# Chuanming-Liu/DAzimSurfTomo

Hardware: AMD Instinct MI355X
Metric: FMM traveltime fields/sec (256^2 grid, 16 periods) + LSQR SpMV HBM GB/s (higher is better)
Workload: dtype f32

## Files before the change

dazimsurftomo_amd/csrc/rays.hip:

```cpp
#include <cmath>
#include <chrono>
#include <unistd.h>

#include "dazim_internal.h"

#include <rocprim/device/device_scan.hpp>
#include <rocprim/device/device_radix_sort.hpp>

namespace {

constexpr int GDX = 5, GDZ = 5;
constexpr int RM = DAZIM_RMAX;
constexpr float EARTH = 6371.0f;
constexpr float FTOL = 1e-4f;

struct RayArgs {
  dazim_geom g;
  int nx, ny, nz, kmax;
  long nray;
  const int *field;
  const float *rcx, *rcz;
  const float *scx, *scz;
  const int *period;
  const int *kidx;
  const float *veln;
  const float *ttn;
  const int *tslot;
  int tsh;
  long fstride;
  const int *fdone;
  int *defer_mark;
  int max_quads;
  int sweeps;
  const float *ttnr;
  const int *nstsr;
  const dazim_refbox *boxes;
  const float *vels;
  const double *svs, *svp, *srho;
  unsigned nvx_magic;
  const double *skern;
  const float *lsen;
  double r_dnx, r_dnz, r_dnxr, r_dnzr, r_dvx, r_dvz, r_e2dnx, r_e2dnxr;
  float dplh;
  float *dsurf;
  int *status;
  int *rbflag;
  long *count;
  int *nlist;
  unsigned short *lcell;
  float *lval;
  float *fdm_scratch;
  int LK;
  int lcap;
  const unsigned *perm;
  unsigned *qcount;
  float2 *pts;
  int *npts;
  int pcap;
  int dense;
  long *countd;
  int keep_small;
  const long *rowptr;
  float *val;
  int *col;
};

__device__ __forceinline__ float dz_sinf(float x) {
  if (!(x > 0.0f && x < 3.1415927f)) return (float)sin((double)x);
  const double y = (double)x - 1.5707963267948966192;
  const double y2 = y * y;
  double p = -1.5619206968586226e-16;
  p = fma(p, y2, 4.7794773323873853e-14);
  p = fma(p, y2, -1.1470745597729725e-11);
  p = fma(p, y2, 2.0876756987868099e-09);
  p = fma(p, y2, -2.7557319223985891e-07);
  p = fma(p, y2, 2.4801587301587302e-05);
  p = fma(p, y2, -1.3888888888888889e-03);
  p = fma(p, y2, 4.1666666666666664e-02);
  p = fma(p, y2, -0.5);
  p = fma(p, y2, 1.0);
  return (float)p;
}

__device__ __forceinline__ void step_azimuth(float x0, float z0, float x1, float z1, float &c2psi, float &s2psi) {
  const float PI_F = 3.1415926535898f;
  const float evtlat = (PI_F / 2 - x0) * 180.0f / PI_F, evtlon = z0 * 180.0f / PI_F;
  const float stalat = (PI_F / 2 - x1) * 180.0f / PI_F, stalon = z1 * 180.0f / PI_F;
  const double pi = (double)3.1415926535898f;
  const float piby2 = (float)(pi / (double)2.f);
  const double rad = (double)2.f * pi / (double)360.f;
  const double sph = (double)(1.0f / 298.257f);
  const double scolat = (double)piby2 - atan((1. - sph) * (1. - sph) * tan((double)stalat * rad));
  const double ecolat = (double)piby2 - atan((1. - sph) * (1. - sph) * tan((double)evtlat * rad));
  const double slon = (double)stalon * rad, elon = (double)evtlon * rad;
  const double a = sin(scolat) * cos(slon), b = sin(scolat) * sin(slon), c = cos(scolat);
  const double dd = sin(elon), ee = -cos(elon), cc = cos(ecolat);
  const double gg = -cc * ee, hh = cc * dd, kk = -sin(ecolat);
  const double rhs1 = (a - dd) * (a - dd) + (b - ee) * (b - ee) + c * c - (double)2.f;
  const double rhs2 = (a - gg) * (a - gg) + (b - hh) * (b - hh) + (c - kk) * (c - kk) - (double)2.f;
  double daz = atan2(rhs1, rhs2);
  if (daz < 0.0) daz = daz + 2 * pi;
  float az = (float)(daz / rad);
  if (fabsf(az - 360.f) < .00001f) az = 0.0f;
  const float rgpsi = az / 180 * PI_F;
  c2psi = (float)cos((double)(2.0f * rgpsi));
  s2psi = (float)sin((double)(2.0f * rgpsi));
}

__device__ __forceinline__ float divr(float x, double rd) { return (float)((double)x * rd); }

__device__ __forceinline__ void basis(float v, float b[4]) {
  const float om = 1.0f - v;
  b[0] = om * om * om / 6.0f;
  b[1] = (4.0f - 6.0f * (v * v) + 3.0f * (v * v * v)) / 6.0f;
  b[2] = (1.0f + 3.0f * v + 3.0f * (v * v) - 3.0f * (v * v * v)) / 6.0f;
  b[3] = v * v * v / 6.0f;
}

__device__ __forceinline__ float div6(float x) { return divr(x, 1.0 / 6.0); }
__device__ __forceinline__ float basis1(float v, int i) {
  const float om = 1.0f - v;
  const float n0 = om * om * om;
  const float n1 = 4.0f - 6.0f * (v * v) + 3.0f * (v * v * v);
  const float n2 = 1.0f + 3.0f * v + 3.0f * (v * v) - 3.0f * (v * v * v);
  const float n3 = v * v * v;
  return div6(i == 0 ? n0 : (i == 1 ? n1 : (i == 2 ? n2 : n3)));
}

__device__ __forceinline__ float vel_at(const dazim_geom &g, const float *veln, int ipx, int ipz, float drx, float drz,
                                        double rdnx, double rdnz) {
  float vel = 0.0f;
#pragma unroll
  for (int l = 1; l <= 2; l++)
#pragma unroll
    for (int m = 1; m <= 2; m++) {
      float produ = (1.0f - fabsf(divr((float)(m - 1) * g.dnz - drz, rdnz)));
      produ = produ * (1.0f - fabsf(divr((float)(l - 1) * g.dnx - drx, rdnx)));
      if (ipz - 1 + m <= g.nnz && ipx - 1 + l <= g.nnx && ipz - 1 + m >= 1 && ipx - 1 + l >= 1)
        vel = vel + veln[(size_t)(ipx - 2 + l) * g.nnz + (ipz - 2 + m)] * produ;
    }
  return vel;
}

__device__ __forceinline__ float bilin_cell(const dazim_geom &g, const float *veln, int cx, int cz, float px, float pz,
                                            double rdnx, double rdnz) {
  const float drx = (px - g.gox) - (float)(cx - 1) * g.dnx;
  const float drz = (pz - g.goz) - (float)(cz - 1) * g.dnz;
  float biv = 0.0f;
#pragma unroll
  for (int i = 1; i <= 2; i++)
#pragma unroll
    for (int j = 1; j <= 2; j++) {
      const float produ = (1.0f - fabsf(divr((float)(i - 1) * g.dnx - drx, rdnx))) *
                          (1.0f - fabsf(divr((float)(j - 1) * g.dnz - drz, rdnz)));
      biv = biv + veln[(size_t)(cx - 2 + i) * g.nnz + (cz - 2 + j)] * produ;
    }
  return biv;
}

__global__ void k_row_kernels(long n, int kmax, long ncol, const float *__restrict__ vels, const double *__restrict__ svs,
                              const double *__restrict__ svp, const double *__restrict__ srho, double *__restrict__ out) {
  const long i = (long)blockIdx.x * blockDim.x + threadIdx.x;
  if (i >= n) return;
  const long k = i / (kmax * ncol), c = i % ncol;
  out[i] = dz_row_kernel(vels[k * ncol + c], svs[i], svp[i], srho[i]);
}

__global__ void k_ray_keys(long nray, const int *__restrict__ field, const float *__restrict__ scx, const float *__restrict__ scz,
                           const float *__restrict__ rcx, const float *__restrict__ rcz, float inv_dmax, int dbits,
                           unsigned *__restrict__ keys, unsigned *__restrict__ iota, const int *__restrict__ order) {
  const long i = (long)blockIdx.x * blockDim.x + threadIdx.x;
  if (i >= nray) return;
  const int f = field[i];
  const float dx = scx[f] - rcx[i], dz = (scz[f] - rcz[i]) * __sinf(rcx[i]);
  const float d = sqrtf(dx * dx + dz * dz) * inv_dmax;
  const unsigned dmaxq = (1u << dbits) - 1u;
  unsigned q = d >= 1.0f ? dmaxq : (unsigned)(d * (float)dmaxq);
  keys[i] = ((unsigned)(order ? order[f] : f) << dbits) | (dmaxq - q);
  iota[i] = (unsigned)i;
}

constexpr int GP_COUNT = 8, GP_EMIT = 16;
constexpr int RAYS_MINW = 4;
constexpr int RPW_MAX = 64 / GP_COUNT;
__device__ __forceinline__ void cbar() { asm volatile("" ::: "memory"); }

template <bool EMIT, bool AZIM, bool TILED, bool MAP>
__global__ __launch_bounds__(64, AZIM ? 2 : RAYS_MINW) void rays_kernel(RayArgs A_) {
  using ArgP = const __attribute__((address_space(4))) RayArgs *;
  auto launder = [](ArgP p) {
    int z;
    asm volatile("v_mov_b32 %0, 0" : "=v"(z));
    return (ArgP)((const __attribute__((address_space(4))) char *)p + __builtin_amdgcn_readfirstlane(z));
  };
  ArgP Ap = launder((ArgP)__builtin_amdgcn_kernarg_segment_ptr());
#define A (*Ap)
#define RAYS_ARGS_FRESH Ap = launder(Ap)
  constexpr int GP = EMIT ? GP_EMIT : GP_COUNT;
  constexpr int RPW = 64 / GP;
  constexpr int LPR = 16 / GP;
  constexpr int LSTEP = 4 / LPR;
  constexpr unsigned GMASK = (1u << GP) - 1u;
  extern __shared__ __attribute__((aligned(16))) unsigned short s_lists[];
  dazim_geom g;
  g.nvx = A.g.nvx; g.nvz = A.g.nvz; g.nnx = A.g.nnx; g.nnz = A.g.nnz;
  g.gox = A.g.gox; g.goz = A.g.goz; g.dnx = A.g.dnx; g.dnz = A.g.dnz; g.dvx = A.g.dvx; g.dvz = A.g.dvz;
  const int lane = threadIdx.x, grp = lane / GP, gl = lane & (GP - 1);
  const int lm = gl & 3, l0 = gl >> 2;
  const int nnx = g.nnx, nnz = g.nnz, nvx = g.nvx, nvz = g.nvz, ldf = nvz + 2, nf = ldf * (nvx + 2);
  constexpr int NG = AZIM ? 3 : 1;
  const unsigned nvx_magic = A.nvx_magic;
  const int LC = A.lcap;
  unsigned short *s_list = s_lists + (size_t)grp * LC;
  float *gfdm = A.fdm_scratch + ((size_t)blockIdx.x * RPW + grp) * nf * NG;
  float *gfdmc = gfdm + nf, *gfdms = gfdm + 2 * nf;
  const float gox = g.gox, goz = g.goz, dnx = g.dnx, dnz = g.dnz, dvx = g.dvx, dvz = g.dvz;
  const double rdnx = A.r_dnx, rdnz = A.r_dnz, rdnxr = A.r_dnxr, rdnzr = A.r_dnzr, rdvx = A.r_dvx, rdvz = A.r_dvz;
  const unsigned gmask_shift = grp * GP;
  const long nquad = (A.nray + RPW - 1) / RPW;
  const int nxcd = (gridDim.x % 8 == 0) ? 8 : 1;
  unsigned *qcnt = A.qcount + (EMIT ? 8 : 0);
  int chunk = (int)(blockIdx.x % nxcd);
  int traced = 0;
  for (;;) {
    RAYS_ARGS_FRESH;
    long quad = -1;
    if (lane == 0) {
      for (int tried = 0; tried < nxcd; tried++) {
        const long lo = nquad * chunk / nxcd, hi = nquad * (chunk + 1) / nxcd;
        const long b = lo < hi ? (long)atomicAdd(&qcnt[chunk], 1u) : hi;
        if (lo + b < hi) {
          quad = lo + b;
          break;
        }
        if (!EMIT && A.sweeps > 1 && lo < hi && b < (hi - lo) * A.sweeps) {
          quad = lo + b % (hi - lo);
          break;
        }
        chunk = (chunk + 1) % nxcd;
      }
    }
    quad = ((long)__shfl((int)(quad >> 32), 0) << 32) | (unsigned)__shfl((int)quad, 0);
    chunk = __shfl(chunk, 0);
    if (quad < 0) break;
    const long slot = quad * RPW + grp;
    if (!EMIT && A.defer_mark) {
      if (!A.defer_mark[quad]) continue;
      if (A.fdone) {
        const int fq = slot < A.nray ? A.field[A.perm ? (long)A.perm[slot] : slot] : -1;
        const int st = fq >= 0 ? __hip_atomic_load(A.fdone + fq, __ATOMIC_ACQUIRE, __HIP_MEMORY_SCOPE_AGENT) : 1;
        if (__ballot(st != 1) != 0) continue;
        __builtin_amdgcn_fence(__ATOMIC_ACQUIRE, "agent");
      }
      if (A.max_quads > 0 && traced >= A.max_quads) break;
      int mine = 0;
      if (lane == 0) mine = __hip_atomic_exchange(A.defer_mark + quad, 0, __ATOMIC_RELAXED, __HIP_MEMORY_SCOPE_AGENT);
      mine = __shfl(mine, 0);
      if (!mine) continue;
      traced++;
      if (lane == 0) atomicAdd(&A.qcount[18], 1u);
    }
    if (slot >= A.nray) continue;
    const long ray = A.perm ? (long)A.perm[slot] : slot;
    const int f = A.field[ray];
    const float scx = A.scx[f], scz = A.scz[f], rcx = A.rcx[ray], rcz = A.rcz[ray];
    const float *veln = A.veln + (size_t)(A.period[f] - 1) * nnx * nnz;
    const float *ttn = TILED ? A.ttn + (size_t)(A.tslot ? A.tslot[f] : f) * A.fstride : A.ttn + (size_t)f * nnx * nnz;
    const int tsh = TILED ? A.tsh : 0;
    auto tnode = [&](int x0, int z0) -> float {
      return TILED ? ttn[dz_tile_x(x0, tsh) + dz_tile_z(z0)] : ttn[(size_t)x0 * nnz + z0];
    };
    const float *ttnr = A.ttnr + (size_t)f * RM * RM;
    const int *nstsr = A.nstsr + (size_t)f * RM * RM;
    const dazim_refbox bx = A.boxes[f];
    const int saved = EMIT ? A.nlist[ray] : -1;
    if (saved < 0)
      for (int i = gl; i < nf * NG; i += GP) gfdm[i] = 0.0f;
    cbar();
    int status = 0, rb = 0;
    if (!EMIT) {
      int irx = (int)divr(rcx - gox, rdnx) + 1, irz = (int)divr(rcz - goz, rdnz) + 1;
      if (irx < 1 || irx > nnx || irz < 1 || irz > nnz) status = DAZIM_E_RECEIVER_OUTSIDE;
      if (!status) {
        if (irx == nnx) irx--;
        if (irz == nnz) irz--;
        const int isx = (int)divr(scx - gox, rdnx) + 1, isz = (int)divr(scz - goz, rdnz) + 1;
        float sred = ((scx - rcx) * EARTH) * ((scx - rcx) * EARTH);
        const float e2 = (scz - rcz) * EARTH * dz_sinf(rcx);
        sred = sqrtf(sred + e2 * e2);
        bool sw = sred < A.dplh;
        if (isx == irx && isz == irz) sw = true;
        float trr;
        if (sw) {
          const float vs = bilin_cell(g, veln, isx, isz, scx, scz, rdnx, rdnz);
          const float vr = bilin_cell(g, veln, irx, irz, rcx, rcz, rdnx, rdnz);
          trr = 2.0f * sred / (vs + vr);
        } else {
          const float drx = (rcx - gox) - (float)(irx - 1) * dnx;
          const float drz = (rcz - goz) - (float)(irz - 1) * dnz;
          trr = 0.0f;
#pragma unroll
          for (int k = 1; k <= 2; k++)
#pragma unroll
            for (int l = 1; l <= 2; l++) {
              const float produ = (1.0f - fabsf(divr((float)(l - 1) * dnz - drz, rdnz))) *
                                  (1.0f - fabsf(divr((float)(k - 1) * dnx - drx, rdnx)));
              trr = trr + tnode(irx - 2 + k, irz - 2 + l) * produ;
            }
        }
        if (gl == 0) A.dsurf[ray] = trr;
      }
    }
    const float goxr = bx.goxr, gozr = bx.gozr, dnxr = bx.dnxr, dnzr = bx.dnzr;
    const int nnxr = bx.nnxr, nnzr = bx.nnzr;
    const int isx = (int)divr(scx - goxr, rdnxr) + 1, isz = (int)divr(scz - gozr, rdnzr) + 1;
    const float dpl = 0.5f * A.dplh;
    int ipx = (int)divr(rcx - gox, rdnx) + 1, ipz = (int)divr(rcz - goz, rdnz) + 1;
    if (ipx < 1 || ipx >= nnx || ipz < 1 || ipz >= nnz) status = DAZIM_E_RECEIVER_OUTSIDE;
    if (!status && saved < 0) {
      float x0 = rcx, z0 = rcz;
      float sinx0 = dz_sinf(x0);
      int sw = 0;
      float sred = ((scx - x0) * EARTH) * ((scx - x0) * EARTH);
      float e2 = (scz - z0) * EARTH * sinx0;
      sred = sqrtf(sred + e2 * e2);
      if (sred < 2.0f * dpl) sw = 1;
      int ipxr = (int)divr(rcx - goxr, rdnxr) + 1, ipzr = (int)divr(rcz - gozr, rdnzr) + 1;
      auto in_refined = [&](int px, int pz) -> int {
        if (px < 1 || px >= nnxr || pz < 1 || pz >= nnzr) return 0;
        const int *sp = nstsr + (size_t)(px - 1) * RM + (pz - 1);
        if (sp[0] != 0 || sp[1] != 0) return 0;
        if (sp[RM] != 0 || sp[RM + 1] != 0) return 0;
        return 1;
      };
      int igref = in_refined(ipxr, ipzr);
      if (sw == 0 && igref == 1 && ipxr == isx && ipzr == isz) sw = 1;
      const bool keep_pts = !EMIT && A.pts != nullptr && gl == 0;
      float2 *rp = A.pts ? A.pts + (size_t)ray * A.pcap : nullptr;
      int np = 1;
      if (keep_pts) {
        rp[0] = make_float2(rcx, rcz);
        if (sw == 1) { if (A.pcap > 1) rp[1] = make_float2(scx, scz); np = 2; }
      }
      int cbx = -100, cbz = -100;
      float acc[LPR], accc[LPR], accs[LPR];
#pragma unroll
      for (int q = 0; q < LPR; q++) acc[q] = accc[q] = accs[q] = 0.0f;
      auto flush = [&]() {
        if (cbx > -100) {
#pragma unroll
          for (int q = 0; q < LPR; q++) {
            const int fi = (cbx + lm) * ldf + (cbz + l0 + q * LSTEP);
            gfdm[fi] = acc[q];
            if (AZIM) { gfdmc[fi] = accc[q]; gfdms[fi] = accs[q]; }
          }
        }
      };
      float tc00, tc01, tc10, tc11, tr00 = 0.0f, tr01 = 0.0f, tr10 = 0.0f, tr11 = 0.0f;
      auto load_corner_times = [&]() {
        if (TILED) {
          const int x0 = dz_tile_x(ipx - 1, tsh), x1 = dz_tile_x(ipx, tsh), z0 = dz_tile_z(ipz - 1), z1 = dz_tile_z(ipz);
          tc00 = ttn[x0 + z0]; tc01 = ttn[x0 + z1]; tc10 = ttn[x1 + z0]; tc11 = ttn[x1 + z1];
        } else {
          const float *t = ttn + (size_t)(ipx - 1) * nnz + (ipz - 1);
          tc00 = t[0]; tc01 = t[1]; tc10 = t[nnz]; tc11 = t[nnz + 1];
        }
        if (ipxr >= 1 && ipxr < nnxr && ipzr >= 1 && ipzr < nnzr) {
          const float *u = ttnr + (size_t)(ipxr - 1) * RM + (ipzr - 1);
          tr00 = u[0]; tr01 = u[1]; tr10 = u[RM]; tr11 = u[RM + 1];
        }
      };
      load_corner_times();
      bool carry = false;
      float vel_c = 0.0f, vi_c = 0.0f, wi_c[LPR];
#pragma unroll
      for (int q = 0; q < LPR; q++) wi_c[q] = 0.0f;
      const long maxrp = (long)nnx * nnz;
      for (long j = 1; j <= maxrp; j++) {
        if (sw == 1) break;
        float dtx, dtz;
        if (igref == 1) {
          dtx = tr10 - tr00;
          dtx = dtx + tr11 - tr01;
          dtx = divr(dtx, A.r_e2dnxr);
          dtz = tr01 - tr00;
          dtz = dtz + tr11 - tr10;
          dtz = dtz / (2.0f * EARTH * sinx0 * dnzr);
        } else {
          dtx = tc10 - tc00;
          dtx = dtx + tc11 - tc01;
          dtx = divr(dtx, A.r_e2dnx);
          dtz = tc01 - tc00;
          dtz = dtz + tc11 - tc10;
          dtz = dtz / (2.0f * EARTH * sinx0 * dnz);
        }
        const float rd1 = sqrtf(dtx * dtx + dtz * dtz);
        float x1 = x0 - dpl * dtx / (EARTH * rd1);
        float z1 = z0 - dpl * dtz / (EARTH * sinx0 * rd1);
        const int ipxo = ipx, ipzo = ipz;
        ipxr = (int)divr(x1 - goxr, rdnxr) + 1;
        ipzr = (int)divr(z1 - gozr, rdnzr) + 1;
        igref = in_refined(ipxr, ipzr);
        ipx = (int)divr(x1 - gox, rdnx) + 1;
        ipz = (int)divr(z1 - goz, rdnz) + 1;
        float sinx1 = dz_sinf(x1);
        sred = ((scx - x1) * EARTH) * ((scx - x1) * EARTH);
        e2 = (scz - z1) * EARTH * sinx1;
        sred = sqrtf(sred + e2 * e2);
        sw = 0;
        if (sred < 2.0f * dpl) sw = 1;
        if (sw == 0 && igref == 1 && ipxr == isx && ipzr == isz) sw = 1;
        bool clipx = false;
        if (ipx < 1) { x1 = gox; ipx = 1; rb = 1; clipx = true; }
        if (ipx >= nnx) { x1 = gox + (float)(nnx - 1) * dnx; ipx = nnx - 1; rb = 1; clipx = true; }
        if (ipz < 1) { z1 = goz; ipz = 1; rb = 1; }
        if (ipz >= nnz) { z1 = goz + (float)(nnz - 1) * dnz; ipz = nnz - 1; rb = 1; }
        load_corner_times();
        if (keep_pts) {
          if (np < A.pcap) rp[np] = make_float2(x1, z1);
          np++;
          if (sw == 1) {
            if (np < A.pcap) rp[np] = make_float2(scx, scz);
            np++;
          }
        }
        if (clipx) sinx1 = dz_sinf(x1);
        float c2psi = 0.0f, s2psi = 0.0f;
        if (AZIM) step_azimuth(x0, z0, x1, z1, c2psi, s2psi);
        const int ivx = (ipx - 1) / GDX + 1, ivz = (ipz - 1) / GDZ + 1;
        const int ivxo = (ipxo - 1) / GDX + 1, ivzo = (ipzo - 1) / GDZ + 1;
        int nhp = 0, chp0 = 0, chp1 = 0;
        float vr0 = 1.0f, vr1 = 1.0f, vr2 = 1.0f;
        if (ivx != ivxo) {
          nhp = 1;
          const float xi = (ivx > ivxo) ? gox + (float)(ivx - 1) * dvx : gox + (float)ivx * dvx;
          vr0 = (xi - x0) / (x1 - x0);
          chp0 = 1;
        }
        if (ivz != ivzo) {
          const float zi = (ivz > ivzo) ? goz + (float)(ivz - 1) * dvz : goz + (float)ivz * dvz;
          const float r = (zi - z0) / (z1 - z0);
          if (nhp == 0) {
            vr0 = r;
            chp0 = 2;
          } else if (r >= vr0) {
            vr1 = r;
            chp1 = 2;
          } else {
            vr1 = vr0;
            chp1 = chp0;
            vr0 = r;
            chp0 = 2;
          }
          nhp++;
        }
        nhp++;
        if (nhp == 1) vr0 = 1.0f;
        if (nhp == 2) vr1 = 1.0f;
        float drx, drz;
        float vel = vel_c, vi = vi_c, wi[LPR];
#pragma unroll
        for (int q = 0; q < LPR; q++) wi[q] = wi_c[q];
        if (__builtin_expect(__ballot(!carry) != 0, 0)) {
          drx = (x0 - gox) - (float)(ipxo - 1) * dnx;
          drz = (z0 - goz) - (float)(ipzo - 1) * dnz;
          vel = vel_at(g, veln, ipxo, ipzo, drx, drz, rdnx, rdnz);
          drx = (x0 - gox) - (float)(ivxo - 1) * dvx;
          drz = (z0 - goz) - (float)(ivzo - 1) * dvz;
          vi = basis1(divr(drx, rdvx), lm);
#pragma unroll
          for (int q = 0; q < LPR; q++) wi[q] = basis1(divr(drz, rdvz), l0 + q * LSTEP);
        }
        int ivxt = ivxo, ivzt = ivzo;
        bool endsame = false;
        for (int k = 1; k <= nhp; k++) {
          const float velo = vel, vio = vi;
          float wio[LPR];
#pragma unroll
          for (int q = 0; q < LPR; q++) wio[q] = wi[q];
          if (k > 1) {
            const int cp = (k == 2) ? chp0 : chp1;
            if (cp == 1) ivxt = ivx;
            else if (cp == 2) ivzt = ivz;
          }
          const float vrk = (k == 1) ? vr0 : (k == 2 ? vr1 : vr2);
          const float vrp = (k == 2) ? vr0 : vr1;
          const float rigz = z0 + vrk * (z1 - z0);
          const float rigx = x0 + vrk * (x1 - x0);
          const int ipxt = (int)divr(rigx - gox, rdnx) + 1, ipzt = (int)divr(rigz - goz, rdnz) + 1;
          endsame = rigx == x1 && rigz == z1 && ipxt == ipx && ipzt == ipz && ivxt == ivx && ivzt == ivz;
          drx = (rigx - gox) - (float)(ipxt - 1) * dnx;
          drz = (rigz - goz) - (float)(ipzt - 1) * dnz;
          vel = vel_at(g, veln, ipxt, ipzt, drx, drz, rdnx, rdnz);
          drx = (rigx - gox) - (float)(ivxt - 1) * dvx;
          drz = (rigz - goz) - (float)(ivzt - 1) * dvz;
          vi = basis1(divr(drx, rdvx), lm);
#pragma unroll
          for (int q = 0; q < LPR; q++) wi[q] = basis1(divr(drz, rdvz), l0 + q * LSTEP);
          const float dinc = (k == 1) ? vrk * dpl : (vrk - vrp) * dpl;
          const int nbx = ivxt - 1, nbz = ivzt - 1;
          if (nbx != cbx || nbz != cbz) {
            flush();
            cbar();
            cbx = nbx;
            cbz = nbz;
#pragma unroll
            for (int q = 0; q < LPR; q++) {
              const int fi = (cbx + lm) * ldf + (cbz + l0 + q * LSTEP);
              acc[q] = gfdm[fi];
              if (AZIM) { accc[q] = gfdmc[fi]; accs[q] = gfdms[fi]; }
            }
          }
#pragma unroll
          for (int q = 0; q < LPR; q++) {
            const float rdc1 = vi * wi[q] / (vel * vel);
            const float rdc2 = vio * wio[q] / (velo * velo);
            float r1 = -(rdc1 + rdc2) * dinc / 2.0f;
            acc[q] = r1 + acc[q];
            if (AZIM) {
              r1 = -(rdc1 * c2psi + rdc2 * c2psi) * dinc / 2.0f;
              accc[q] = r1 + accc[q];
              r1 = -(rdc1 * s2psi + rdc2 * s2psi) * dinc / 2.0f;
              accs[q] = r1 + accs[q];
            }
          }
        }
        carry = endsame;
        vel_c = vel;
        vi_c = vi;
#pragma unroll
        for (int q = 0; q < LPR; q++) wi_c[q] = wi[q];
        x0 = x1;
        z0 = z1;
        sinx0 = sinx1;
      }
      flush();
      if (keep_pts) A.npts[ray] = np <= A.pcap ? np : -1;
    }
    cbar();
    if (!EMIT && gl == 0) {
      if (A.pts && status) A.npts[ray] = 0;
      A.status[ray] = status;
      A.rbflag[ray] = rb;
    }
    int nlist = 0;
    if (saved >= 0) {
      nlist = saved;
      const size_t o = (size_t)ray * A.LK, ov = o * NG;
      for (int i = gl; i < nlist; i += GP) {
        const int c = A.lcell[o + i];
        const int jj = (int)__umulhi((unsigned)c, nvx_magic) + 1, kk = c - (jj - 1) * nvx + 1;
        s_list[i] = (unsigned short)c;
        gfdm[kk * ldf + jj] = A.lval[ov + i];
        if (AZIM) {
          gfdmc[kk * ldf + jj] = A.lval[ov + A.LK + i];
          gfdms[kk * ldf + jj] = A.lval[ov + 2 * A.LK + i];
        }
      }
    } else if (!status) {
      for (int base = 0; base < nvz * nvx; base += GP) {
        const int c = base + gl;
        bool keep = false;
        if (c < nvz * nvx) {
          const int jj = (int)__umulhi((unsigned)c, nvx_magic) + 1, kk = c - (jj - 1) * nvx + 1;
          keep = fabsf(gfdm[kk * ldf + jj]) >= FTOL;
        }
        const unsigned m = (unsigned)((__ballot(keep) >> gmask_shift) & GMASK);
        const int pos = nlist + __popc(m & ((1u << gl) - 1u));
        if (keep && pos < LC) s_list[pos] = (unsigned short)c;
        nlist += __popc(m);
      }
    }
    cbar();
    if (!EMIT) {
      const size_t o = (size_t)ray * A.LK, ov = o * NG;
      if (nlist <= A.LK)
        for (int i = gl; i < nlist; i += GP) {
          const int c = s_list[i];
          const int jj = (int)__umulhi((unsigned)c, nvx_magic) + 1, kk = c - (jj - 1) * nvx + 1;
          A.lcell[o + i] = (unsigned short)c;
          A.lval[ov + i] = gfdm[kk * ldf + jj];
          if (AZIM) {
            A.lval[ov + A.LK + i] = gfdmc[kk * ldf + jj];
            A.lval[ov + 2 * A.LK + i] = gfdms[kk * ldf + jj];
          }
        }
      if (gl == 0) A.nlist[ray] = (status || nlist <= A.LK) ? (status ? 0 : nlist) : -1;
    }
    const size_t ncol = (size_t)A.nx * A.ny;
    const int kslot = A.kidx[f] - 1;
    long cnt = 0;
    const long rstart = EMIT ? A.rowptr[ray] : 0;
    const int nparpi = nvx * nvz * (A.nz - 1);
    const int nlay = MAP ? 1 : A.nz - 1;
    const int bstride = MAP ? A.kmax * nvx * nvz : nparpi;
    const int poff = MAP ? (A.period[f] - 1) * nvx * nvz : 0;
    const bool lovf = nlist > LC;
    const int ntot = lovf ? nvz * nvx : nlist;
    long cntd = 0;
    int jjL = 1, kkL = 1;
    if (A.dense) {
      int clast = -1;
      if (!lovf) {
        if (nlist > 0) clast = s_list[nlist - 1];
      } else {
        for (int base = ((nvz * nvx - 1) / GP) * GP; base >= 0 && clast < 0; base -= GP) {
          const int c = base + gl;
          bool k2 = false;
          if (c < nvz * nvx) {
            const int jj = (int)__umulhi((unsigned)c, nvx_magic) + 1, kk = c - (jj - 1) * nvx + 1;
            k2 = fabsf(gfdm[kk * ldf + jj]) >= FTOL;
          }
          const unsigned m2 = (unsigned)((__ballot(k2) >> gmask_shift) & GMASK);
          if (m2) clast = base + (31 - __clz(m2));
        }
      }
      if (clast >= 0) { jjL = (int)__umulhi((unsigned)clast, nvx_magic) + 1; kkL = clast - (jjL - 1) * nvx + 1; }
    }
    constexpr int RC = 8;
    const bool rowcache = !lovf && ntot <= RC * GP && (MAP || A.skern != nullptr) && !A.dense;
    if (rowcache) {
      int sidx[RC], cbase[RC], fidx[RC];
#pragma unroll
      for (int i = 0; i < RC; i++) {
        const int li = i * GP + gl;
        const int c = li < ntot ? (int)s_list[li] : 0;
        const int jj = (int)__umulhi((unsigned)c, nvx_magic) + 1, kk = c - (jj - 1) * nvx + 1;
        sidx[i] = jj * (nvx + 2) + kk;
        cbase[i] = (jj - 1) * nvx + kk;
        fidx[i] = kk * ldf + jj;
      }
      for (int blk = 0; blk < NG; blk++) {
        float fdv[RC];
        const float *fsrc = blk == 0 ? gfdm : (blk == 1 ? gfdmc : gfdms);
#pragma unroll
        for (int i = 0; i < RC; i++) fdv[i] = (i * GP + gl < ntot) ? fsrc[fidx[i]] : 0.0f;
        for (int k = 1; k <= nlay; k++) {
          const size_t sk = ((size_t)(k - 1) * A.kmax + kslot) * ncol;
          const int nk = blk * bstride + poff + (k - 1) * nvz * nvx;
#pragma unroll
          for (int i = 0; i < RC; i++) {
            if (i * GP >= ntot) break;
            const bool cell = i * GP + gl < ntot;
            float rowv = 0.0f;
            bool keep = false;
            if (cell) {
              if (MAP) rowv = fdv[i];
              else if (blk == 0) rowv = (float)(A.skern[sk + sidx[i]] * (double)fdv[i]);
              else rowv = A.lsen[sk + sidx[i]] * fdv[i];
              keep = A.keep_small ? (rowv != 0.0f) : (fabsf(rowv) > FTOL);
            }
            const unsigned m = (unsigned)((__ballot(keep) >> gmask_shift) & GMASK);
            if (EMIT && keep) {
              const long pos = rstart + cnt + __popc(m & ((1u << gl) - 1u));
              A.val[pos] = rowv;
              A.col[pos] = nk + cbase[i] - 1;
            }
            cnt += __popc(m);
          }
        }
      }
    } else
    for (int blk = 0; blk < NG; blk++)
      for (int k = 1; k <= nlay; k++) {
        for (int base = 0; base < ntot; base += GP) {
          const int li = base + gl;
          bool keep = false, keepd = false;
          float rowv = 0.0f;
          int nn = 0;
          bool cell = li < ntot;
          int c = 0;
          if (cell) c = lovf ? li : s_list[li];
          const int jj = (int)__umulhi((unsigned)c, nvx_magic) + 1, kk = c - (jj - 1) * nvx + 1;
          if (cell && lovf) cell = fabsf(gfdm[kk * ldf + jj]) >= FTOL;
          if (cell && MAP) {
            rowv = (blk == 0 ? gfdm : (blk == 1 ? gfdmc : gfdms))[kk * ldf + jj];
            keep = A.keep_small ? (rowv != 0.0f) : (fabsf(rowv) > FTOL);
            nn = blk * bstride + poff + (jj - 1) * nvx + kk;
          } else if (cell) {
            const size_t si = ((size_t)(k - 1) * A.kmax + kslot) * ncol + (size_t)jj * (nvx + 2) + kk;
            if (blk == 0) {
              const float fd = gfdm[kk * ldf + jj];
              double r;
              if (A.skern) {
                r = A.skern[si] * (double)fd;
              } else {
                const float v = A.vels[((size_t)(k - 1) * A.ny + jj) * A.nx + kk];
// ... 52 lines not shown
  const int *period = nullptr, *kidx = nullptr, *nstsr = nullptr, *field = nullptr;
  const dazim_refbox *boxes = nullptr;
  const double *svs = nullptr, *svp = nullptr, *srho = nullptr;
  int64_t nray = 0;
  float *dsurf = nullptr;
  dazim_csr **G = nullptr;
  int64_t *nnz_out = nullptr;
  int *n_boundary = nullptr;
  bool map = false, azim = false;
  struct StreamSwap {
    dazim_ctx *c; hipStream_t main; bool on = false;
    void restore() { if (on) { c->stream = main; on = false; } }
    ~StreamSwap() {
      if (on) (void)hipStreamSynchronize(c->stream);
      restore();
    }
  } swap;
  struct {
    DzBuf<float> vels, scx, scz, veln, ttn, ttnr, rcx, rcz, dsurf, lsen;
    DzBuf<int> period, kidx, nstsr, field;
    DzBuf<dazim_refbox> boxes;
    DzBuf<double> svs, svp, srho;
  } d;
  struct Arrays {
    dazim_ctx *c; int64_t *rp = nullptr; float *v = nullptr; int *cl = nullptr; int64_t nnz = 0, cap_nnz = 0; bool keep = false;
    ~Arrays() { if (!keep) { dz_big_put(c, rp); dz_big_put(c, v); dz_big_put(c, cl); } }
  } arrays, arrays_d;
  dazim_geom g;
  bool joint = false, tiled = false, overlap = false, twin = false;
  size_t nn = 0, nr = 0, ncol = 0, nk = 0, nr1 = 0, lds = 0;
  int64_t res_rows = 0, res_nnz = 0;
  long nwg = 0;
  double overlap_tail_s = 0.0;
  RayArgs A;
  explicit RayBuild(dazim_ctx *c) : ctx(c), swap{c, c ? c->stream : nullptr}, arrays{c}, arrays_d{c} {}
  int check() {
    if (!ctx || !G) return DAZIM_E_BAD_ARG;
    joint = map ? azim : lsen != nullptr;
    if (map) nz = 2;
    if (map && dz_opt(ctx, "rays.dense_twin", 0) != 0)
      return dz_fail(ctx, DAZIM_E_BAD_ARG, "dazim_rays_build_G_maps: option rays.dense_twin serves the 3-D program's diagnostics only");
    if (dazim_geometry(nx, ny, goxd, gozd, dvxd, dvzd, &g)) return dz_fail(ctx, DAZIM_E_BAD_ARG, "bad grid");
    if (nray < 0 || nfield < 1 || nz < 2 || kmax < 1 || (size_t)g.nvx * g.nvz > 65535u) return dz_fail(ctx, DAZIM_E_BAD_ARG, "bad arguments to dazim_rays_build_G");
    tiled = ttn == nullptr;
    if (tiled && (!ctx->fields.tiled || ctx->fields.nfield != nfield || ctx->fields.nnx != g.nnx || ctx->fields.nnz != g.nnz))
      return dz_fail(ctx, DAZIM_E_BAD_ARG, "dazim_rays_build_G: ttn is NULL and the last dazim_fmm_batch call did not keep %d fields of this grid inside the library (call it with ttn = NULL)", nfield);
    if (!scx || !scz || !period || !veln || !ttnr || !nstsr || !boxes || !dsurf ||
        (!map && (!vels || !svs || !svp || !srho)) || (nray > 0 && (!field || !rcx || !rcz)))
      return dz_fail(ctx, DAZIM_E_BAD_ARG, "dazim_rays_build_G: NULL array (the refined fields ttnr, nstsr and boxes of dazim_fmm_batch are required)");
    DZ_HIP(hipSetDevice(ctx->device));
    return 0;
  }
  int decide_overlap() {
    overlap = (bool)ctx->fmm_finish && tiled && ctx->fields.fdone && nray > 0;
    if (overlap && ctx->aux_epilogue && ctx->comm && ((DzComm *)ctx->comm)->nccl) overlap = false;
    if (overlap)
      for (const void *q : {(const void *)vels, (const void *)scx, (const void *)scz, (const void *)period, (const void *)veln,
                            (const void *)ttnr, (const void *)nstsr, (const void *)boxes, (const void *)field, (const void *)rcx,
                            (const void *)rcz, (const void *)svs, (const void *)svp, (const void *)srho, (const void *)dsurf,
                            (const void *)kidx, (const void *)lsen})
        if (q && !dz_is_device_ptr(q)) overlap = false;
    if (!overlap) { const int rcf = dz_fmm_finish(ctx); if (rcf) return rcf; }
    if (overlap) {
      DZ_HIP(hipStreamWaitEvent(ctx->stream3, ctx->ev_pre, 0));
      ctx->stream = ctx->stream3;
      swap.on = true;
    }
    return dz_join_aux(ctx);
  }
  int stage_inputs() {
    nn = (size_t)g.nnx * g.nnz; nr = (size_t)RM * RM; ncol = (size_t)nx * ny;
    int rc;
    if (!map && (rc = d.vels.init(ctx, vels, (size_t)nz * ncol, true, false))) return rc;
    if ((rc = d.scx.init(ctx, scx, nfield, true, false)) || (rc = d.scz.init(ctx, scz, nfield, true, false)) ||
        (rc = d.period.init(ctx, period, nfield, true, false)) || (rc = d.kidx.init(ctx, kidx ? kidx : period, nfield, true, false)) ||
        (rc = d.veln.init(ctx, veln, nn * kmax, true, false)) || (!tiled && (rc = d.ttn.init(ctx, ttn, nn * nfield, true, false))) ||
        (rc = d.ttnr.init(ctx, ttnr, nr * nfield, true, false)) || (rc = d.nstsr.init(ctx, nstsr, nr * nfield, true, false)) ||
        (rc = d.boxes.init(ctx, boxes, nfield, true, false)) || (rc = d.field.init(ctx, field, nray, true, false)) ||
        (rc = d.rcx.init(ctx, rcx, nray, true, false)) || (rc = d.rcz.init(ctx, rcz, nray, true, false)))
      return rc;
    nk = (size_t)nz * kmax * ncol;
    if (!map && ((rc = d.svs.init(ctx, svs, nk, true, false)) || (rc = d.svp.init(ctx, svp, nk, true, false)) ||
                  (rc = d.srho.init(ctx, srho, nk, true, false))))
      return rc;
    if ((rc = d.dsurf.init(ctx, dsurf, nray, false, true))) return rc;
    if (joint && !map && (rc = d.lsen.init(ctx, lsen, (size_t)(nz - 1) * kmax * ncol, true, false))) return rc;
    if ((rc = dz_check_range(ctx, d.period.dev, nfield, 1, kmax, "period_idx"))) return rc;
    if ((rc = dz_check_range(ctx, d.kidx.dev, nfield, 1, kmax, "kernel_idx"))) return rc;
    return dz_check_range(ctx, d.field.dev, nray, 0, nfield - 1, "field_of_ray");
  }
  int kernel_constants() {
    int rc;
    A.g = g;
    A.nx = nx; A.ny = ny; A.nz = nz; A.kmax = kmax;
    A.nray = nray;
    A.field = d.field.dev; A.rcx = d.rcx.dev; A.rcz = d.rcz.dev; A.scx = d.scx.dev; A.scz = d.scz.dev;
    A.period = d.period.dev; A.kidx = d.kidx.dev; A.veln = d.veln.dev; A.ttn = d.ttn.dev; A.ttnr = d.ttnr.dev;
    A.tslot = nullptr; A.tsh = 0; A.fstride = (long)nn;
    if (tiled) {
      A.ttn = reinterpret_cast<const float *>(ctx->fields.tiled);
      A.tslot = ctx->fields.tslot; A.tsh = ctx->fields.tsh; A.fstride = ctx->fields.stride;
    }
    ctx->ksec["rays.tiled_fields"] = tiled ? 1.0 : 0.0;
    ctx->ksec["rays.map"] = map ? 1.0 : 0.0;
    ctx->ksec["rays.overlap"] = overlap ? 1.0 : 0.0;
    A.fdone = overlap ? ctx->fields.fdone : nullptr;
    A.defer_mark = nullptr; A.max_quads = 0; A.sweeps = 1;
    A.nstsr = d.nstsr.dev; A.boxes = d.boxes.dev; A.vels = d.vels.dev; A.svs = d.svs.dev; A.svp = d.svp.dev; A.srho = d.srho.dev;
    A.lsen = joint && !map ? d.lsen.dev : nullptr;
    A.skern = nullptr;
    {
      const unsigned dv = (unsigned)g.nvx;
      A.nvx_magic = (unsigned)((0x100000000ull + dv - 1) / dv);
      for (unsigned c = 0; c < 65536u; c++)
        if ((unsigned)(((unsigned long long)c * A.nvx_magic) >> 32) != c / dv) return dz_fail(ctx, DAZIM_E_BAD_ARG, "internal: reciprocal of nvx");
    }
    if (!map && dz_opt(ctx, "rays.skern", 1) != 0) {
      double *pk;
      if ((rc = dz_scratch(ctx, "rays.skern", nk, &pk))) return rc;
      hipLaunchKernelGGL(k_row_kernels, dim3((unsigned)((nk + 255) / 256)), dim3(256), 0, ctx->stream, (long)nk, kmax, (long)ncol,
                         d.vels.dev, d.svs.dev, d.svp.dev, d.srho.dev, pk);
      DZ_HIP(hipGetLastError());
      A.skern = pk;
    }
    {
      float dpl = g.dnx * EARTH;
      float rd1 = g.dnz * EARTH * sinf(g.gox);
      if (rd1 < dpl) dpl = rd1;
      rd1 = g.dnz * EARTH * sinf(g.gox + (float)(g.nnx - 1) * g.dnx);
      if (rd1 < dpl) dpl = rd1;
      A.dplh = dpl;
    }
    {
      const float dnxr = g.dvx / (float)(GDX * 8), dnzr = g.dvz / (float)(GDZ * 8);
      const float e2dnx = 2.0f * EARTH * g.dnx, e2dnxr = 2.0f * EARTH * dnxr;
      A.r_dnx = 1.0 / (double)g.dnx;   A.r_dnz = 1.0 / (double)g.dnz;
      A.r_dnxr = 1.0 / (double)dnxr;   A.r_dnzr = 1.0 / (double)dnzr;
      A.r_dvx = 1.0 / (double)g.dvx;   A.r_dvz = 1.0 / (double)g.dvz;
      A.r_e2dnx = 1.0 / (double)e2dnx; A.r_e2dnxr = 1.0 / (double)e2dnxr;
    }
    return 0;
  }
  int scratch() {
    int rc;
    nr1 = (size_t)(nray > 0 ? nray : 1);
    if ((rc = dz_scratch(ctx, "rays.status", nr1, &A.status))) return rc;
    if ((rc = dz_scratch(ctx, "rays.rb", nr1, &A.rbflag))) return rc;
    if ((rc = dz_scratch(ctx, "rays.count", (size_t)(nray + 1), &A.count))) return rc;
    A.lcap = g.nvx * g.nvz <= 4096 ? 512 : 1024;
    if (dz_opt(ctx, "rays.lcap", 0) >= 16 && dz_opt(ctx, "rays.lcap", 0) <= 8192) A.lcap = dz_opt(ctx, "rays.lcap", 0);
    if (A.lcap > g.nvx * g.nvz) A.lcap = g.nvx * g.nvz;
    A.LK = A.lcap;
    A.keep_small = dz_opt(ctx, "rays.keep_small", 0) != 0 ? 1 : 0;
    A.pts = nullptr; A.npts = nullptr; A.pcap = 0;
    if (dz_opt(ctx, "rays.keep_paths", 0) != 0) {
      A.pcap = 4 * (g.nnx + g.nnz) + 16;
      if ((rc = dz_scratch(ctx, "rays.pts", nr1 * (size_t)A.pcap, &A.pts))) return rc;
      if ((rc = dz_scratch(ctx, "rays.npts", nr1, &A.npts))) return rc;
      DZ_HIP(hipMemsetAsync(A.npts, 0, nr1 * 4, ctx->stream));
    }
    ctx->ksec["rays.path_cap"] = A.pcap;
    ctx->ksec["rays.path_rays"] = A.pts ? (double)nray : 0.0;
    twin = dz_opt(ctx, "rays.dense_twin", 0) != 0 && !A.keep_small;
    A.dense = twin ? 2 : 0;
    A.countd = nullptr;
    if (twin) {
      if ((rc = dz_scratch(ctx, "rays.countd", (size_t)(nray + 1), &A.countd))) return rc;
      DZ_HIP(hipMemsetAsync(A.countd, 0, (size_t)(nray + 1) * 8, ctx->stream));
    }
    if ((rc = dz_scratch(ctx, "rays.nlist", nr1, &A.nlist))) return rc;
    if ((rc = dz_scratch(ctx, "rays.lcell", nr1 * A.LK, &A.lcell))) return rc;
    if ((rc = dz_scratch(ctx, "rays.lval", nr1 * A.LK * (joint ? 3 : 1), &A.lval))) return rc;
    res_rows = (int64_t)g.nvx * g.nvz * (map ? kmax : nz - 1) * (joint ? 3 : 1);
    res_nnz = (map ? 5 : 7) * res_rows;
    if (dz_opt(ctx, "csr.reserve_rows", 0) > res_rows) res_rows = dz_opt(ctx, "csr.reserve_rows", 0);
    if (dz_opt(ctx, "csr.reserve_nnz", 0) > res_nnz) res_nnz = dz_opt(ctx, "csr.reserve_nnz", 0);
    if ((rc = dz_big_get(ctx, (size_t)(nray + res_rows + 1), &arrays.rp))) return rc;
    A.dsurf = d.dsurf.dev;
    A.rowptr = (const long *)arrays.rp; A.val = nullptr; A.col = nullptr;
    return 0;
  }
  template <int I> static const void *kernel_no() { return (const void *)rays_kernel<(I & 8) != 0, (I & 4) != 0, (I & 2) != 0, (I & 1) != 0>; }
  const void *kern(bool emit) const {
    static const void *const tab[16] = {kernel_no<0>(),  kernel_no<1>(),  kernel_no<2>(),  kernel_no<3>(), kernel_no<4>(),  kernel_no<5>(),
                                        kernel_no<6>(),  kernel_no<7>(),  kernel_no<8>(),  kernel_no<9>(), kernel_no<10>(), kernel_no<11>(),
                                        kernel_no<12>(), kernel_no<13>(), kernel_no<14>(), kernel_no<15>()};
    return tab[(emit ? 8 : 0) + (joint ? 4 : 0) + (tiled ? 2 : 0) + (map ? 1 : 0)];
  }
  int launch(bool emit, const RayArgs &R, long nwg_) {
    RayArgs args = R;
    void *params[] = {&args};
    DZ_HIP(hipLaunchKernel(kern(emit), dim3((unsigned)nwg_), dim3(64), params, lds, ctx->stream));
    return 0;
  }
  int launch_shape() {
    lds = (size_t)A.lcap * 2 * RPW_MAX + 16;
    DZ_HIP(hipFuncSetAttribute(kern(false), hipFuncAttributeMaxDynamicSharedMemorySize, (int)lds));
    DZ_HIP(hipFuncSetAttribute(kern(true), hipFuncAttributeMaxDynamicSharedMemorySize, (int)lds));
    int per_cu = (int)(160 * 1024 / (lds + 256));
    {
      int occ = 0;
      const void *kf = kern(false);
      if (hipOccupancyMaxActiveBlocksPerMultiprocessor(&occ, kf, 64, lds) == hipSuccess && occ > 0 && occ < per_cu) per_cu = occ;
    }
    if (per_cu > 16) per_cu = 16;
    if (per_cu < 1) return dz_fail(ctx, DAZIM_E_BAD_ARG, "inversion grid too large for the LDS cell lists");
    if (dz_opt(ctx, "rays.wg_per_cu", 0) > 0 && dz_opt(ctx, "rays.wg_per_cu", 0) < per_cu) per_cu = dz_opt(ctx, "rays.wg_per_cu", 0);
    nwg = (long)ctx->num_cu * per_cu;
    if (nwg > (nray + RPW_MAX - 1) / RPW_MAX) nwg = (nray + RPW_MAX - 1) / RPW_MAX;
    if (nwg >= 8) nwg -= nwg % 8;
    if (nwg < 1) nwg = 1;
    return dz_scratch(ctx, "rays.fdm", (size_t)nwg * RPW_MAX * (g.nvx + 2) * (g.nvz + 2) * (joint ? 3 : 1), &A.fdm_scratch);
  }
  int sort_rays() {
    int rc;
    A.perm = nullptr;
    if (nray >= 64 && nray < (1ll << 32) && dz_opt(ctx, "rays.sort", 1) != 0) {
      int fbits = 1;
      while ((1ll << fbits) < nfield) fbits++;
      const int dbits = 32 - fbits > 12 ? 12 : 32 - fbits;
      if (dbits >= 4) {
        unsigned *k0, *k1, *v0, *v1;
        if ((rc = dz_scratch(ctx, "rays.sortbuf", (size_t)nray * 4 + 16, &k0))) return rc;
        k1 = k0 + nray; v0 = k1 + nray; v1 = v0 + nray;
        const float ex = (float)g.nnx * g.dnx, ez = (float)g.nnz * g.dnz;
        const float inv_dmax = 1.0f / sqrtf(ex * ex + ez * ez);
        hipLaunchKernelGGL(k_ray_keys, dim3((unsigned)((nray + 255) / 256)), dim3(256), 0, ctx->stream, (long)nray, d.field.dev, d.scx.dev,
                           d.scz.dev, d.rcx.dev, d.rcz.dev, inv_dmax, dbits, k0, v0, overlap ? A.tslot : (const int *)nullptr);
        size_t tb = 0;
        DZ_HIP(rocprim::radix_sort_pairs(nullptr, tb, k0, k1, v0, v1, (size_t)nray, 0, fbits + dbits, ctx->stream));
        void *tmp;
        if ((rc = dz_scratch(ctx, "rays.sorttmp", tb + 256, &tmp))) return rc;
        DZ_HIP(rocprim::radix_sort_pairs(tmp, tb, k0, k1, v0, v1, (size_t)nray, 0, fbits + dbits, ctx->stream));
        A.perm = v1;
      }
    }
    if ((rc = dz_scratch(ctx, "rays.qcount", 32, &A.qcount))) return rc;
    DZ_HIP(hipMemsetAsync(A.qcount, 0, 128, ctx->stream));
    if (overlap) {
      const size_t nq = (size_t)((nray + RPW_MAX - 1) / RPW_MAX) + 8;
      if ((rc = dz_scratch(ctx, "rays.defer", nq, &A.defer_mark))) return rc;
      DZ_HIP(hipMemsetAsync(A.defer_mark, 0, nq * 4, ctx->stream));
    }
    return 0;
  }
  int count_pass() { return nray > 0 ? launch(false, A, nwg) : 0; }
  int count_passes_beside_eikonal() {
    int rc;
    const auto t_poll0 = std::chrono::steady_clock::now();
    auto fmm_over = [&]() {
      const bool over = hipEventQuery(ctx->ev_f1) == hipSuccess;
      if (!over) (void)hipGetLastError();
      return over;
    };
    if (ctx->fields.hprog && ctx->fields.total_tasks > 0) {
      const unsigned slack = ctx->fields.nwg / 4 + 8 * 16;
      const unsigned total = ctx->fields.total_tasks;
      const unsigned want = total > slack ? total - slack : 0;
      for (;;) {
        unsigned have = 0;
        for (int c = 0; c < 8; c++) have += ctx->fields.hprog[c];
        if (have >= want || fmm_over()) break;
        if (std::chrono::steady_clock::now() - t_poll0 > std::chrono::seconds(120)) break;
        usleep(50);
      }
    }
    const unsigned nquad_all = (unsigned)((nray + RPW_MAX - 1) / RPW_MAX);
    unsigned pending = nquad_all, *h_traced = nullptr;
    { void *hp; if ((rc = dz_pinned(ctx, "rays.host_pending", 64, &hp))) return rc; h_traced = (unsigned *)hp; }
    DZ_HIP(hipMemsetAsync(A.defer_mark, 1, (size_t)nquad_all * 4, ctx->stream));
    int npass = 0;
    bool collected = false, ev0_set = false;
    unsigned left_by_first = 0;
    int rcf = 0;
    while (pending > 0) {
      const bool last = fmm_over();
      if (last && !collected) {
        swap.restore();
        DZ_HIP(hipStreamSynchronize(ctx->stream3));
        rcf = dz_fmm_finish(ctx);
        collected = true;
        if (rcf) break;
        if (npass == 0) (void)hipEventRecord(ctx->ev_r1, ctx->stream);
        (void)hipEventRecord(ctx->ev0, ctx->stream);
        ev0_set = true;
      }
      long nwg_pass = nwg;
      A.max_quads = 0;
      A.sweeps = collected ? 1 : 3;
      if (collected) A.fdone = nullptr;
      DZ_HIP(hipMemsetAsync(A.qcount, 0, 32, ctx->stream));
      if ((rc = launch(false, A, nwg_pass))) return rc;
      if (!collected) DZ_HIP(hipEventRecord(ctx->ev_r1, ctx->stream));
      DZ_HIP(hipMemcpyAsync(h_traced, A.qcount + 18, 4, hipMemcpyDeviceToHost, ctx->stream));
      DZ_HIP(hipStreamSynchronize(ctx->stream));
      const unsigned before = pending;
      pending = collected ? 0u : nquad_all - *h_traced;
      if (npass == 0) left_by_first = pending;
      npass++;
      if (pending > 0 && pending == before) usleep(100);
    }
    swap.restore();
    if (!collected) rcf = dz_fmm_finish(ctx);
    DZ_HIP(hipStreamSynchronize(ctx->stream3));
    if (rcf) return rcf;
    ctx->ksec["rays.passes"] = npass;
// ... 157 lines not shown
```

Measured before the change: 54370.

## Streamline ray-step loop: skip refined-grid work far from source, carry rdc terms

In the ray-tracing step loop, refined-grid cell lookup and its corner-time loads now run only when some lane in the wavefront is within a distance threshold of the source. The per-step carried state is reduced from vel/vi/wi to the precomputed rdc products. An unchecked interior velocity interpolation is used when all lanes are inside the grid, and the B-spline basis is evaluated with fewer operations. It also adds optional asm markers for inspecting the ISA, and a plain_step option to disable the shortcut. The distance-threshold skip relies on a geometric bound and could change results if that bound is wrong.

```diff
diff --git a/dazimsurftomo_amd/csrc/rays.hip b/dazimsurftomo_amd/csrc/rays.hip
--- a/dazimsurftomo_amd/csrc/rays.hip
+++ b/dazimsurftomo_amd/csrc/rays.hip
@@ -8,6 +8,12 @@
 #include <rocprim/device/device_radix_sort.hpp>
 
 namespace {
+
+#ifdef DZ_RAYS_MARK
+#define RAYS_MARK(i) asm volatile("; MARK " #i ::: "memory")
+#else
+#define RAYS_MARK(i)
+#endif
 
 constexpr int GDX = 5, GDZ = 5;
 constexpr int RM = DAZIM_RMAX;
@@ -59,6 +65,7 @@
   int pcap;
   int dense;
   long *countd;
+  int plain_step;
   int keep_small;
   const long *rowptr;
   float *val;
@@ -119,12 +126,12 @@
 
 __device__ __forceinline__ float div6(float x) { return divr(x, 1.0 / 6.0); }
 __device__ __forceinline__ float basis1(float v, int i) {
-  const float om = 1.0f - v;
-  const float n0 = om * om * om;
-  const float n1 = 4.0f - 6.0f * (v * v) + 3.0f * (v * v * v);
-  const float n2 = 1.0f + 3.0f * v + 3.0f * (v * v) - 3.0f * (v * v * v);
-  const float n3 = v * v * v;
-  return div6(i == 0 ? n0 : (i == 1 ? n1 : (i == 2 ? n2 : n3)));
+  const float w = i == 0 ? 1.0f - v : v;
+  const float t2 = w * w, t3 = t2 * w;
+  const float p = i == 1 ? 4.0f : 1.0f + 3.0f * v;
+  const float c = i == 1 ? -6.0f : 3.0f, d = i == 1 ? 3.0f : -3.0f;
+  const float n = (p + c * t2) + d * t3;
+  return div6((i == 0 || i == 3) ? t3 : n);
 }
 
 __device__ __forceinline__ float vel_at(const dazim_geom &g, const float *veln, int ipx, int ipz, float drx, float drz,
@@ -138,6 +145,19 @@
       produ = produ * (1.0f - fabsf(divr((float)(l - 1) * g.dnx - drx, rdnx)));
       if (ipz - 1 + m <= g.nnz && ipx - 1 + l <= g.nnx && ipz - 1 + m >= 1 && ipx - 1 + l >= 1)
         vel = vel + veln[(size_t)(ipx - 2 + l) * g.nnz + (ipz - 2 + m)] * produ;
+    }
+  return vel;
+}
+__device__ __forceinline__ float vel_at_interior(const dazim_geom &g, const float *veln, int ipx, int ipz, float drx, float drz,
+                                                 double rdnx, double rdnz) {
+  float vel = 0.0f;
+#pragma unroll
+  for (int l = 1; l <= 2; l++)
+#pragma unroll
+    for (int m = 1; m <= 2; m++) {
+      float produ = (1.0f - fabsf(divr((float)(m - 1) * g.dnz - drz, rdnz)));
+      produ = produ * (1.0f - fabsf(divr((float)(l - 1) * g.dnx - drx, rdnx)));
+      vel = vel + veln[(size_t)(ipx - 2 + l) * g.nnz + (ipz - 2 + m)] * produ;
     }
   return vel;
 }
@@ -365,19 +385,25 @@
           const float *t = ttn + (size_t)(ipx - 1) * nnz + (ipz - 1);
           tc00 = t[0]; tc01 = t[1]; tc10 = t[nnz]; tc11 = t[nnz + 1];
         }
+      };
+      auto load_refined_corner_times = [&]() {
         if (ipxr >= 1 && ipxr < nnxr && ipzr >= 1 && ipzr < nnzr) {
           const float *u = ttnr + (size_t)(ipxr - 1) * RM + (ipzr - 1);
           tr00 = u[0]; tr01 = u[1]; tr10 = u[RM]; tr11 = u[RM + 1];
         }
       };
       load_corner_times();
+      load_refined_corner_times();
       bool carry = false;
-      float vel_c = 0.0f, vi_c = 0.0f, wi_c[LPR];
-#pragma unroll
-      for (int q = 0; q < LPR; q++) wi_c[q] = 0.0f;
+      float rdc[LPR];
+#pragma unroll
+      for (int q = 0; q < LPR; q++) rdc[q] = 0.0f;
+      float fart = __builtin_inff();
+      int nnx_in = 0, nnz_in = 0;
       const long maxrp = (long)nnx * nnz;
       for (long j = 1; j <= maxrp; j++) {
         if (sw == 1) break;
+        RAYS_MARK(0);
         float dtx, dtz;
         if (igref == 1) {
           dtx = tr10 - tr00;
@@ -397,24 +423,36 @@
         const float rd1 = sqrtf(dtx * dtx + dtz * dtz);
         float x1 = x0 - dpl * dtx / (EARTH * rd1);
         float z1 = z0 - dpl * dtz / (EARTH * sinx0 * rd1);
+        RAYS_MARK(1);
         const int ipxo = ipx, ipzo = ipz;
-        ipxr = (int)divr(x1 - goxr, rdnxr) + 1;
-        ipzr = (int)divr(z1 - gozr, rdnzr) + 1;
-        igref = in_refined(ipxr, ipzr);
+        const float sdx = scx - x1, sdz = scz - z1;
+        bool srcell = false;
+        if (__ballot(!(fabsf(sdx) > fart || fabsf(sdz) > fart)) != 0) {
+          ipxr = (int)divr(x1 - goxr, rdnxr) + 1;
+          ipzr = (int)divr(z1 - gozr, rdnzr) + 1;
+          igref = in_refined(ipxr, ipzr);
+          srcell = igref == 1 && ipxr == isx && ipzr == isz;
+          load_refined_corner_times();
+        } else {
+          igref = 0;
+        }
         ipx = (int)divr(x1 - gox, rdnx) + 1;
         ipz = (int)divr(z1 - goz, rdnz) + 1;
+        RAYS_MARK(2);
         float sinx1 = dz_sinf(x1);
-        sred = ((scx - x1) * EARTH) * ((scx - x1) * EARTH);
-        e2 = (scz - z1) * EARTH * sinx1;
+        sred = (sdx * EARTH) * (sdx * EARTH);
+        e2 = sdz * EARTH * sinx1;
         sred = sqrtf(sred + e2 * e2);
         sw = 0;
         if (sred < 2.0f * dpl) sw = 1;
-        if (sw == 0 && igref == 1 && ipxr == isx && ipzr == isz) sw = 1;
+        if (srcell) sw = 1;
+        RAYS_MARK(3);
         bool clipx = false;
         if (ipx < 1) { x1 = gox; ipx = 1; rb = 1; clipx = true; }
         if (ipx >= nnx) { x1 = gox + (float)(nnx - 1) * dnx; ipx = nnx - 1; rb = 1; clipx = true; }
         if (ipz < 1) { z1 = goz; ipz = 1; rb = 1; }
         if (ipz >= nnz) { z1 = goz + (float)(nnz - 1) * dnz; ipz = nnz - 1; rb = 1; }
+        RAYS_MARK(4);
         load_corner_times();
         if (keep_pts) {
           if (np < A.pcap) rp[np] = make_float2(x1, z1);
@@ -427,6 +465,7 @@
         if (clipx) sinx1 = dz_sinf(x1);
         float c2psi = 0.0f, s2psi = 0.0f;
         if (AZIM) step_azimuth(x0, z0, x1, z1, c2psi, s2psi);
+        RAYS_MARK(5);
         const int ivx = (ipx - 1) / GDX + 1, ivz = (ipz - 1) / GDZ + 1;
         const int ivxo = (ipxo - 1) / GDX + 1, ivzo = (ipzo - 1) / GDZ + 1;
         int nhp = 0, chp0 = 0, chp1 = 0;
@@ -457,27 +496,27 @@
         nhp++;
         if (nhp == 1) vr0 = 1.0f;
         if (nhp == 2) vr1 = 1.0f;
+        RAYS_MARK(6);
         float drx, drz;
-        float vel = vel_c, vi = vi_c, wi[LPR];
-#pragma unroll
-        for (int q = 0; q < LPR; q++) wi[q] = wi_c[q];
         if (__builtin_expect(__ballot(!carry) != 0, 0)) {
           drx = (x0 - gox) - (float)(ipxo - 1) * dnx;
           drz = (z0 - goz) - (float)(ipzo - 1) * dnz;
-          vel = vel_at(g, veln, ipxo, ipzo, drx, drz, rdnx, rdnz);
+          const float vel = vel_at(g, veln, ipxo, ipzo, drx, drz, rdnx, rdnz);
           drx = (x0 - gox) - (float)(ivxo - 1) * dvx;
           drz = (z0 - goz) - (float)(ivzo - 1) * dvz;
-          vi = basis1(divr(drx, rdvx), lm);
-#pragma unroll
-          for (int q = 0; q < LPR; q++) wi[q] = basis1(divr(drz, rdvz), l0 + q * LSTEP);
-        }
+          const float vi = basis1(divr(drx, rdvx), lm);
+#pragma unroll
+          for (int q = 0; q < LPR; q++) rdc[q] = vi * basis1(divr(drz, rdvz), l0 + q * LSTEP) / (vel * vel);
+          if (A.plain_step == 0) {
+            fart = (float)((RM - 1) / 8 + 1) * fmaxf(dnx, dnz);
+            nnx_in = nnx;
+            nnz_in = nnz;
+          }
+        }
+        RAYS_MARK(7);
         int ivxt = ivxo, ivzt = ivzo;
         bool endsame = false;
         for (int k = 1; k <= nhp; k++) {
-          const float velo = vel, vio = vi;
-          float wio[LPR];
-#pragma unroll
-          for (int q = 0; q < LPR; q++) wio[q] = wi[q];
           if (k > 1) {
             const int cp = (k == 2) ? chp0 : chp1;
             if (cp == 1) ivxt = ivx;
@@ -491,14 +530,20 @@
           endsame = rigx == x1 && rigz == z1 && ipxt == ipx && ipzt == ipz && ivxt == ivx && ivzt == ivz;
           drx = (rigx - gox) - (float)(ipxt - 1) * dnx;
           drz = (rigz - goz) - (float)(ipzt - 1) * dnz;
-          vel = vel_at(g, veln, ipxt, ipzt, drx, drz, rdnx, rdnz);
+          const bool inner = ipxt >= 1 && ipxt < nnx_in && ipzt >= 1 && ipzt < nnz_in;
+          endsame = endsame && inner;
+          float vel;
+          if (__builtin_expect(__ballot(!inner) == 0, 1)) vel = vel_at_interior(g, veln, ipxt, ipzt, drx, drz, rdnx, rdnz);
+          else vel = vel_at(g, veln, ipxt, ipzt, drx, drz, rdnx, rdnz);
           drx = (rigx - gox) - (float)(ivxt - 1) * dvx;
           drz = (rigz - goz) - (float)(ivzt - 1) * dvz;
-          vi = basis1(divr(drx, rdvx), lm);
+          const float vi = basis1(divr(drx, rdvx), lm);
+          float wi[LPR];
 #pragma unroll
           for (int q = 0; q < LPR; q++) wi[q] = basis1(divr(drz, rdvz), l0 + q * LSTEP);
           const float dinc = (k == 1) ? vrk * dpl : (vrk - vrp) * dpl;
           const int nbx = ivxt - 1, nbz = ivzt - 1;
+          RAYS_MARK(8);
           if (nbx != cbx || nbz != cbz) {
             flush();
             cbar();
@@ -511,10 +556,12 @@
               if (AZIM) { accc[q] = gfdmc[fi]; accs[q] = gfdms[fi]; }
             }
           }
+          RAYS_MARK(9);
 #pragma unroll
           for (int q = 0; q < LPR; q++) {
             const float rdc1 = vi * wi[q] / (vel * vel);
-            const float rdc2 = vio * wio[q] / (velo * velo);
+            const float rdc2 = rdc[q];
+            rdc[q] = rdc1;
             float r1 = -(rdc1 + rdc2) * dinc / 2.0f;
             acc[q] = r1 + acc[q];
             if (AZIM) {
@@ -525,14 +572,12 @@
             }
           }
         }
+        RAYS_MARK(10);
         carry = endsame;
-        vel_c = vel;
-        vi_c = vi;
-#pragma unroll
-        for (int q = 0; q < LPR; q++) wi_c[q] = wi[q];
         x0 = x1;
         z0 = z1;
         sinx0 = sinx1;
+      RAYS_MARK(11);
       }
       flush();
       if (keep_pts) A.npts[ray] = np <= A.pcap ? np : -1;
@@ -891,6 +936,7 @@
     if (A.lcap > g.nvx * g.nvz) A.lcap = g.nvx * g.nvz;
     A.LK = A.lcap;
     A.keep_small = dz_opt(ctx, "rays.keep_small", 0) != 0 ? 1 : 0;
+    A.plain_step = dz_opt(ctx, "rays.plain_step", 0) != 0 ? 1 : 0;
     A.pts = nullptr; A.npts = nullptr; A.pcap = 0;
     if (dz_opt(ctx, "rays.keep_paths", 0) != 0) {
       A.pcap = 4 * (g.nnx + g.nnz) + 16;
```

New measurement: 55560, median of 6. 2.2% higher.
